# decisionforce/pgdrive

Measured on AMD Instinct MI355X. Metric: env-steps/sec (whole node) at 4096 envs x 240 lidar beams, higher is better.
Workload: dtype f32; 1 GPU; C3: 4096 envs/GPU x (1 ego + 16 IDM traffic slots) x 240 lidar beams, PGDrive-v0 maps seeds 1000-1099, uniform(-1,1) actions, auto-reset; step_kernel=k_step: one env per wave, specialised for the default single-agent configuration, envs_per_gpu=4096, global_envs=4096, obs_dim=274, engines_per_gpu=1, env_groups=1, parallelism=env-sharded dp1, no data-path collective, backend=none, steady_state=pre-roll 10000 steps (floor 10000), 1571 timed steps in 3 windows

## Files before the change

### pgdrive_amd/csrc/pgd_localize.h

```cpp
#ifndef PGD_LOCALIZE_H
#define PGD_LOCALIZE_H

DEV int cell_first(int c) { return c & 0xffffff; }
DEV int cell_mid(int c) { return (c & 0xffffff) + (int)((unsigned)c >> 24); }

template <class MV>
DEV float ray_grid(const MV& mv, float px, float py, float dx, float dy, unsigned kinds) {
  const float inv = 1.0f / mv.cell();
  int ix = (int)floorf((px - mv.ox()) * inv), iy = (int)floorf((py - mv.oy()) * inv);
  const int sx = dx > 0.0f ? 1 : -1, sy = dy > 0.0f ? 1 : -1;
  const float big = 3.0e38f;
  const float tdx = dx != 0.0f ? fabsf(mv.cell() / dx) : big, tdy = dy != 0.0f ? fabsf(mv.cell() / dy) : big;
  float tmx = dx != 0.0f ? ((mv.ox() + (ix + (dx > 0.0f ? 1 : 0)) * mv.cell()) - px) / dx : big;
  float tmy = dy != 0.0f ? ((mv.oy() + (iy + (dy > 0.0f ? 1 : 0)) * mv.cell()) - py) / dy : big;
  float best = 1.0f, t_enter = 0.0f;
  for (int it = 0; it < 64; ++it) {
    if (t_enter > best + 0.02f) break;
    if (ix >= 0 && iy >= 0 && ix < mv.gx() && iy < mv.gy()) {
      const int cell = iy * mv.gx() + ix;
      const int k1 = cell_first(mv.cstart[cell + 1]);
      for (int k = cell_mid(mv.cstart[cell]); k < k1; ++k) {
        const pgd_box b = mv.cbox[k];
        if (!((1u << b.kind) & kinds)) continue;
        best = fminf(best, ray_obb(obb_of(b), px, py, dx, dy));
      }
    } else if ((sx > 0 ? ix >= mv.gx() : ix < 0) || (sy > 0 ? iy >= mv.gy() : iy < 0)) {
      break;
    }
    if (tmx < tmy) { t_enter = tmx; tmx += tdx; ix += sx; }
    else { t_enter = tmy; tmy += tdy; iy += sy; }
    if (t_enter > 1.0f) break;
  }
  return best;
}


template <class MV>
DEV int cell_entry(const MV& mv, float px, float py) {
  int cx = (int)floorf((px - mv.ox()) / mv.cell()), cy = (int)floorf((py - mv.oy()) / mv.cell());
  return (cx >= 0 && cy >= 0 && cx < mv.gx() && cy < mv.gy()) ? mv.cstart[cy * mv.gx() + cx] : 0;
}

DEV int get_current_lane(const MapView& mv, const Grp& g, int c, float px, float py, float hx, float hy, int road_cur,
                         int road_next) {
  const int k0 = cell_first(c), k1 = cell_mid(c);
  unsigned best_cur = 0xffffffffu, best_next = 0xffffffffu, best_any = 0xffffffffu;
  const int stride = g.SUB;
  constexpr int NB = 3;
  for (int k = k0 + g.sub; k < k1; k += NB * stride) {
    pgd_box b[NB];
    LaneExt x[NB];
#pragma unroll
    for (int j = 0; j < NB; ++j) {
      int kk = k + j * stride;
      kk = kk < k1 ? kk : k;
      b[j] = mv.cbox[kk];
      x[j] = mv.cext[kk];
    }
#pragma unroll
    for (int j = 0; j < NB; ++j) {
      int kk = k + j * stride;
      if (kk >= k1) continue;
      if (!point_in_obb(obb_of(b[j]), px, py)) continue;
      unsigned key = ((unsigned)(kk - k0) << 16) | (unsigned)b[j].lane;
      bool is_cur = x[j].road == road_cur, is_next = x[j].road == road_next;
      if (!(key < best_any || (is_cur && key < best_cur) || (is_next && key < best_next))) continue;
      float dirx, diry;
      if (x[j].dir == 0.0f) { dirx = x[j].ax; diry = x[j].ay; }
      else { dirx = -x[j].dir * (py - x[j].ay); diry = x[j].dir * (px - x[j].ax); }
      if (!(dirx * hx + diry * hy > 0.0f)) continue;
      best_any = min(best_any, key);
      if (is_cur) best_cur = min(best_cur, key);
      if (is_next) best_next = min(best_next, key);
    }
  }
  best_cur = group_min(best_cur, g);
  best_next = group_min(best_next, g);
  best_any = group_min(best_any, g);
  unsigned pick = best_cur != 0xffffffffu ? best_cur : (road_next < 0 ? best_any : (best_next != 0xffffffffu ? best_next : best_any));
  return pick == 0xffffffffu ? -1 : (int)(pick & 0xffffu);
}

DEV void route_refresh(const MapView& mv, const pgd_spawn& sp, Veh& r) {
  const int rc = sp.ckpt_road[r.ck0], rn = sp.ckpt_road[r.ck1];
  r.road_cur = (uint32_t)rc; r.road_next = (uint32_t)rn;
  r.blk = 0; r.cur_first = 0; r.cur_n = 0; r.next_first = 0; r.next_n = 0;
  if (rc >= 0) {
    const pgd_road& CR = mv.roads()[rc];
    r.blk = CR.block_id; r.cur_first = CR.first_lane; r.cur_n = CR.n_lanes;
  }
  if (rn >= 0) {
    const pgd_road& NR = mv.roads()[rn];
    r.next_first = NR.first_lane; r.next_n = NR.n_lanes;
  }
}

#define PGD_CKPT_END (-32768)
DEV void update_checkpoints(const MapView& mv, const Grp& g, const pgd_spawn& sp, Veh& r, float lon, const int start_node) {
  if (r.ck0 == r.ck1) return;
  if (!(lon < 5.0f)) return;
  unsigned hit = 0xffffffffu;
  const int step = g.SUB;
#ifdef PGD_CKPT_CHAIN
  const int n = sp.n_ckpt;
  const int start_node_ = mv.roads()[mv.lanes[r.lane].road].from;
  for (int k = r.ck1 + g.sub; k < n - 1; k += 4 * step) {
    int v[4];
#pragma unroll
    for (int j = 0; j < 4; ++j) v[j] = sp.ckpt[min(k + j * step, n - 2)];
#pragma unroll
    for (int j = 0; j < 4; ++j)
      if (k + j * step < n - 1 && v[j] == start_node_) hit = min(hit, (unsigned)(k + j * step));
  }
#else
  for (int k = r.ck1 + g.sub; k < PGD_MAX_CKPT; k += 4 * step) {
    int v[4];
#pragma unroll
    for (int j = 0; j < 4; ++j) v[j] = sp.ckpt[min(k + j * step, PGD_MAX_CKPT - 1)];
#pragma unroll
    for (int j = 0; j < 4; ++j)
      if (k + j * step < PGD_MAX_CKPT && v[j] == start_node) hit = min(hit, (unsigned)(k + j * step));
    if (v[3] == PGD_CKPT_END) break;
  }
#endif
  hit = group_min(hit, g);
  if (hit == 0xffffffffu) return;
  const int idx = (int)hit;
  const int n_nodes = sp.n_ckpt;
  r.ck0 = idx;
  r.ck1 = (idx + 1 == n_nodes - 1) ? idx : idx + 1;
  route_refresh(mv, sp, r);
}

template <class MV>
DEV void update_localization(const MV& mv, const Grp& g, const pgd_spawn& sp, Veh& r, float& lon_out, float& lat_out,
                             const pgd_lane& PL) {
  const float s = r.hy, c = r.hx;
  const int road_cur = (int)r.road_cur;
  const int road_next = (r.ck0 == r.ck1) ? -1 : (int)r.road_next;
  PHASE_MARK(16);
  float lon = 0.0f, lat = 0.0f;
  bool stay = false;
  const int cell = cell_entry(mv, r.x, r.y);
  {
    if (PL.road == road_cur) {
      lane_local(PL, r.x, r.y, lon, lat);
      const float hw = 0.5f * PL.width;
      if (PL.dir == 0.0f) {
        stay = lon >= 0.0f && lon <= PL.length && lat <= hw + 0.55f && lat >= (PL.index > 0 ? 0.65f - hw : -hw - 0.55f) &&
               PL.bx * c + PL.by * s > 0.0f;
      } else {
        const int n = (int)(PL.length * 0.25f);
        const float r_in = PL.bx - PL.width - 1.0f;
        if (n >= 1 && r_in > 4.0f) {
          const float seg = PL.length / (float)n;
          const float dev = seg * seg / (4.0f * r_in) * 1.1f + 0.05f;
          float lo = -hw - 0.6f + dev;
          if (PL.index > 0) {
            const float nl = mv.lanes[r.lane - 1].length;
            const int nn = (int)(nl * 0.25f);
            if (nn >= 1) {
              const float nseg = nl / (float)nn;
              lo = fmaxf(lo, 0.6f - hw + nseg * nseg / (4.0f * r_in) * 1.1f + 0.05f);
            }
          }
          const float tx = -PL.dir * (r.y - PL.ay), ty = PL.dir * (r.x - PL.ax);
          stay = lon >= 0.0f && lon <= PL.length && lat <= hw + 0.6f - dev && lat >= lo && tx * c + ty * s > 0.0f;
        }
      }
    }
  }
  int lane = r.lane;
  if (!stay) lane = get_current_lane(mv, g, cell, r.x, r.y, c, s, road_cur, road_next);
  PHASE_MARK(17);
  bool on_lane = lane >= 0;
  if (!on_lane) lane = r.lane;
  r.lane = lane;
  int from_node = PL.pad;
  if (!stay) {
    const pgd_lane& NL = mv.lanes[lane];
    from_node = NL.pad;
    lane_local(NL, r.x, r.y, lon, lat);
  }
  lon_out = lon; lat_out = lat;
  r.lon = lon;
  update_checkpoints(mv, g, sp, r, lon, from_node);
  r.vflags = on_lane ? (r.vflags & ~PGD_F_OFF_LANE) : (r.vflags | PGD_F_OFF_LANE);
  PHASE_MARK(18);
}

template <class MV>
DEV unsigned state_check_part(const MV& mv, const int g_sub, const int g_SUB, const Obb& car) {
  float ex = fabsf(car.ux) * car.hl + fabsf(car.uy) * car.hw, ey = fabsf(car.uy) * car.hl + fabsf(car.ux) * car.hw;
  int cx0 = max((int)floorf((car.cx - ex - mv.ox()) / mv.cell()), 0), cx1 = min((int)floorf((car.cx + ex - mv.ox()) / mv.cell()), mv.gx() - 1);
  int cy0 = max((int)floorf((car.cy - ey - mv.oy()) / mv.cell()), 0), cy1 = min((int)floorf((car.cy + ey - mv.oy()) / mv.cell()), mv.gy() - 1);
  unsigned fl = 0;
  for (int cyb = cy0; cyb <= cy1; cyb += 2)
    for (int cxb = cx0; cxb <= cx1; cxb += 2) {
      int k0[4], pre[5];
      pre[0] = 0;
#pragma unroll
      for (int q = 0; q < 4; ++q) {
        int cx = cxb + (q & 1), cy = cyb + (q >> 1);
        bool in = cx <= cx1 && cy <= cy1;
        int cell = in ? cy * mv.gx() + cx : 0;
        int a = cell_mid(mv.cstart[cell]), b = cell_first(mv.cstart[cell + 1]);
        k0[q] = a;
        pre[q + 1] = pre[q] + (in ? b - a : 0);
      }
      const int n = pre[4];
      for (int f = g_sub; f < n; f += 2 * g_SUB) {
        pgd_box b[2];
        bool have[2];
#pragma unroll
        for (int j = 0; j < 2; ++j) {
          const int fj = f + j * g_SUB;
          have[j] = fj < n;
          const int ff = have[j] ? fj : f;
          const int q = (ff >= pre[1]) + (ff >= pre[2]) + (ff >= pre[3]);
          const int kk = (q == 0 ? k0[0] : q == 1 ? k0[1] : q == 2 ? k0[2] : k0[3]) + ff - (q == 0 ? pre[0] : q == 1 ? pre[1] : q == 2 ? pre[2] : pre[3]);
          b[j] = mv.cbox[kk];
        }
#pragma unroll
        for (int j = 0; j < 2; ++j) {
          if (!have[j]) continue;
          const unsigned bit = b[j].kind == PGD_BOX_WHITE ? PGD_F_ON_WHITE
                               : b[j].kind == PGD_BOX_YELLOW ? PGD_F_ON_YELLOW
                               : b[j].kind == PGD_BOX_BROKEN ? PGD_F_ON_BROKEN : PGD_F_CRASH_SIDEWALK;
          if (fl & bit) continue;
          if (obb_overlap(car, obb_of(b[j]))) fl |= bit;
        }
      }
    }
  return fl;
}
template <class MV>
DEV unsigned state_check(const MV& mv, const Grp& g, const Obb& car) { return group_or(state_check_part(mv, g.sub, g.SUB, car), g); }

struct RouteCtx {
  float drive;
  float positive;
  int clear;
  int lane_road;
};

template <bool AHEAD = false, class MV>
DEV void after_step_vehicle(const pgd_config& cfg, const MV& mv, const Grp& g, const pgd_spawn& sp, const pgd_spawn& sv, Veh& r,
                            bool is_agent, bool with_state_check, RouteCtx& ctx) {
  float lon_v, lat_v;
  const int lane0 = r.lane, first0 = (int)r.cur_first;
  const pgd_lane PL = mv.lanes[lane0];
  pgd_lane L0;
  if (AHEAD && is_agent) L0 = mv.lanes[first0];
  update_localization(mv, g, sp, r, lon_v, lat_v, PL);
  if (is_agent) {
    ctx = RouteCtx{0.0f, 1.0f, 0, -1};
    pgd_lane VL = PL;
    if (!AHEAD || r.lane != lane0) VL = mv.lanes[r.lane];
    ctx.lane_road = VL.road;
    if (!AHEAD || (int)r.cur_first != first0) L0 = mv.lanes[r.cur_first];
    {
      if (VL.dir == 0.0f && VL.ex > 0.0f) {
        const float ca = fabsf(r.hx * VL.bx + r.hy * VL.by), sa = fabsf(r.hy * VL.bx - r.hx * VL.by);
        const float hl = 0.5f * sv.length, hw = 0.5f * sv.width;
        const float e_lat = hw * ca + hl * sa, e_lon = hl * ca + hw * sa;
        ctx.clear = (fabsf(lat_v) + e_lat <= VL.ex && lon_v - e_lon >= 0.0f && lon_v + e_lon <= VL.length) ? 1 : 0;
      }
    }
    unsigned fl = (unsigned)r.vflags;
    fl &= ~(PGD_F_ON_WHITE | PGD_F_ON_YELLOW | PGD_F_ON_BROKEN | PGD_F_CRASH_SIDEWALK | PGD_F_OUT_OF_ROUTE);
    if (with_state_check && !ctx.clear) fl |= state_check(mv, g, Obb{r.x, r.y, r.hx, r.hy, 0.5f * sv.length, 0.5f * sv.width});
    float lon, lat;
    lane_local(L0, r.x, r.y, lon, lat);
    float w = mv.lane_width();
    r.dl = lat + w * 0.5f;
    float range = w * (float)r.cur_n;
    if (r.blk == 'y' || r.blk == 'Y') {
      float sx, sy;
      lane_position(L0, lon, -0.5f * L0.width, sx, sy);
      range = 50.0f * ray_grid(mv, sx, sy, -L0.by * 50.0f, L0.bx * 50.0f, (1u << PGD_BOX_WHITE) | (1u << PGD_BOX_YELLOW));
    }
    r.dr = range - r.dl;
    {
      const bool in_ref = VL.road == (int)r.road_cur;
      float l0, t0;
      lane_local(in_ref ? VL : L0, r.lastx, r.lasty, l0, t0);
      const float l1 = in_ref ? lon_v : lon, t1 = in_ref ? lat_v : lat;
      ctx.positive = (in_ref || (cfg.marl_flags & PGD_MA_PLAIN_REWARD)) ? 1.0f : (mv.roads()[VL.road].negative ? -1.0f : 1.0f);
      const float lateral_factor = cfg.use_lateral ? clipf(1.0f - 2.0f * fabsf(t1) / w, 0.0f, 1.0f) : 1.0f;
      ctx.drive = cfg.driving_reward * (l1 - l0) * lateral_factor * ctx.positive;
    }
    if (r.dr < 0.0f || r.dl < 0.0f) fl |= PGD_F_OUT_OF_ROUTE;
    r.vflags = (int)fl;
    float dist = norm2(r.lastx - r.x, r.lasty - r.y) / 1000.0f;
    r.energy += 3.25f * expf(0.01f * speed_kmh(r.v)) * dist / 100.0f * 1000.0f;
    PHASE_MARK(19);
  }
}

template <class MV>
DEV unsigned state_check_wave(const MV& mv, const Obb& car) {
  const int lane = threadIdx.x;
  float ex = fabsf(car.ux) * car.hl + fabsf(car.uy) * car.hw, ey = fabsf(car.uy) * car.hl + fabsf(car.ux) * car.hw;
  int cx0 = max((int)floorf((car.cx - ex - mv.ox()) / mv.cell()), 0), cx1 = min((int)floorf((car.cx + ex - mv.ox()) / mv.cell()), mv.gx() - 1);
  int cy0 = max((int)floorf((car.cy - ey - mv.oy()) / mv.cell()), 0), cy1 = min((int)floorf((car.cy + ey - mv.oy()) / mv.cell()), mv.gy() - 1);
  unsigned fl = 0;
  for (int cyb = cy0; cyb <= cy1; cyb += 2)
    for (int cxb = cx0; cxb <= cx1; cxb += 2) {
      int k0[4], pre[5];
      pre[0] = 0;
#pragma unroll
      for (int q = 0; q < 4; ++q) {
        int cx = cxb + (q & 1), cy = cyb + (q >> 1);
        bool in = cx <= cx1 && cy <= cy1;
        int cell = in ? cy * mv.gx() + cx : 0;
        int a = cell_mid(mv.cstart[cell]), b = cell_first(mv.cstart[cell + 1]);
        k0[q] = a;
        pre[q + 1] = pre[q] + (in ? b - a : 0);
      }
      for (int f = lane; f < pre[4]; f += WAVE) {
        int q = (f >= pre[1]) + (f >= pre[2]) + (f >= pre[3]);
        int kk = (q == 0 ? k0[0] : q == 1 ? k0[1] : q == 2 ? k0[2] : k0[3]) + f - (q == 0 ? pre[0] : q == 1 ? pre[1] : q == 2 ? pre[2] : pre[3]);
        pgd_box b = mv.cbox[kk];
        unsigned bit = b.kind == PGD_BOX_WHITE ? PGD_F_ON_WHITE
                       : b.kind == PGD_BOX_YELLOW ? PGD_F_ON_YELLOW
                       : b.kind == PGD_BOX_BROKEN ? PGD_F_ON_BROKEN : PGD_F_CRASH_SIDEWALK;
        if (obb_overlap(car, obb_of(b))) fl |= bit;
      }
    }
  unsigned out = 0;
  if (__ballot((fl & PGD_F_ON_WHITE) != 0)) out |= PGD_F_ON_WHITE;
  if (__ballot((fl & PGD_F_ON_YELLOW) != 0)) out |= PGD_F_ON_YELLOW;
  if (__ballot((fl & PGD_F_ON_BROKEN) != 0)) out |= PGD_F_ON_BROKEN;
  if (__ballot((fl & PGD_F_CRASH_SIDEWALK) != 0)) out |= PGD_F_CRASH_SIDEWALK;
  return out;
}

#endif
```

### pgdrive_amd/csrc/pgd_step.h

```cpp
#define WAVE 64
#define MAXV 64

#ifndef PGD_MA_PRIO3
#define PGD_MA_PRIO3 7
#define PGD_MA_PRIO2 5
#define PGD_MA_PRIO1 3
#endif
#ifdef PGD_PROF
#define PROF_BLOCKS 8192
__device__ unsigned long long g_phase_cycles[PROF_BLOCKS * 32];
__shared__ long long s_prof_t0, s_prof_w0;
#define PHASE_MARK(k)                                                                                      \
  do {                                                                                                     \
    if ((int)threadIdx.x == __builtin_ffsll((long long)__ballot(1)) - 1 && blockIdx.x < PROF_BLOCKS) {       \
      long long _now = clock64();                                                                          \
      g_phase_cycles[blockIdx.x * 32 + (k)] += (unsigned long long)(_now - s_prof_t0);                     \
      s_prof_t0 = _now;                                                                                    \
    }                                                                                                      \
  } while (0)
#define PHASE_INIT() do { if (threadIdx.x == 0) { s_prof_t0 = clock64(); s_prof_w0 = wall_clock64(); } } while (0)
#define PHASE_END_AT(k) do { if (threadIdx.x == 0 && blockIdx.x < PROF_BLOCKS) g_phase_cycles[blockIdx.x * 32 + (k)] += (unsigned long long)(wall_clock64() - s_prof_w0); } while (0)
#define PHASE_END() PHASE_END_AT(15)
#elif defined(PGD_EXITAT)
#define PHASE_MARK(k)
// ... 171 lines not shown
  float lk_klat, lk_khead, lk_vt, lk_noise;
  uint32_t lk_tick;
};
template <bool ONE_ENV, bool MARL, bool OBJ, bool STD = false, int FIX = 0, bool LK = false>
__global__ __launch_bounds__(WAVE, PGD_WAVES_PER_SIMD) void k_step(PgdDev d, const float* __restrict__ act, float* __restrict__ reward,
                                                uint8_t* __restrict__ done, uint32_t* __restrict__ flags,
                                                float* __restrict__ obs, const PgdCold cold) {
  if (FIX) write_fixed_config<ONE_ENV, MARL, STD, FIX>(d);

  __shared__ StepUnion U;
  Snap& S = U.step.S;
  ObsScratch& OU = U.step.OU;
  ObsLds& OL = OU.ol;
  SubPose& SUBP = OU.sp;
  __shared__ AgentView s_ag[FUSE_MAX_AGENTS];
  __shared__ int s_flag[WAVE];
  __shared__ int s_hit[WAVE];
  __shared__ int s_aux;
  __shared__ uint8_t s_kind[WAVE];
  const int V = d.V, A = d.A, N = d.N;
  const int lane = threadIdx.x;
  const bool sub_ok = (ONE_ENV ? V : d.epw * V) <= PGD_SUBV;
  const int unit = (int)blockIdx.x + d.unit_off;
  const LaneMap lm = lane_map(d, unit, N);
  const int el = ONE_ENV ? 0 : lm.el, s = lm.s, e = ONE_ENV ? unit : lm.e, base = ONE_ENV ? 0 : lm.base;
  const bool valid = lm.valid, leader = lm.sub == 0;
  const Grp g{lm.sub, d.sub, lm.lead};
  const int slot = base + s;

  PHASE_INIT();
  XMARK(99);
  Veh r;
  RouteCtx ctx{0.0f, 1.0f, 0, -1};
  using MV = typename std::conditional<FIX != 0 && !OBJ, MapViewPre, MapView>::type;
  MV mv;
  const pgd_spawn* sp = nullptr;
  constexpr bool FIXE_K = FIX != 0 && !ONE_ENV && !MARL && !STD;
  constexpr bool REGSP = ONE_ENV || FIXE_K;
  pgd_spawn sl;
  pgd_lane FL;
#define SPV spawn_ref<REGSP>(sl, sp)
  const pgd_scenario* sc = nullptr;
  int ng = 0, ep_steps = 0;
  uint32_t steps_total = 0;
  bool near_env = true;
  int trig_hint = 0;
#ifdef PGD_NO_SUBSTEP
  constexpr bool n_mid_enabled = false;
#else
  constexpr bool n_mid_enabled = true;
#endif
  S.present[lane] = 0;
  s_flag[lane] = 0;
  s_hit[lane] = 0;
  if (lane < PGD_SUBV) SUBP.trav[lane] = 0.0f;
  constexpr bool one_env = ONE_ENV;
  constexpr bool marl = MARL;
  int scen = 0;
  unsigned long long im = 0ull;
  const bool packed = !ONE_ENV && d.pack_obs != 0;
  const bool own_first = FIX == 0 && ONE_ENV && !d.use_imask;
  if (own_first && valid) load_rec(rec_block(d.rec, (size_t)e, V), V, s, r);
  if ((ONE_ENV || (packed && valid)) && d.use_imask) im = d.imask[e];
  if (one_env || valid) scen = d.ei[(size_t)e * PGD_NEI + EI_SCEN];
  constexpr bool LATE_WORDS = MARL && FIX != 0;
  int hint_early = 0;
  if (LATE_WORDS && (one_env || valid)) hint_early = d.ei[(size_t)e * PGD_NEI + EI_NEAR];
  if (valid && !own_first) load_rec(((ONE_ENV || packed) && ((im >> s) & 1ull)) ? rec_block(d.reset_img, (size_t)scen, V) : rec_block(d.rec, (size_t)e, V), V, s, r);
  float2 act_in = make_float2(0.0f, 0.0f);
  constexpr bool ACT_EARLY = ONE_ENV || FIXE_K;
  if (ACT_EARLY && valid && s < A) {
    if (LK) {
      const float* o = cold.lk_obs + ((size_t)e * A + s) * d.D;
      const float2 q0 = *reinterpret_cast<const float2*>(o), q1 = *reinterpret_cast<const float2*>(o + 2);
      act_in = lane_keep_action(cold.seed, cold.env_base + e, q0.x, q0.y, q1.x, q1.y, cold.lk_klat, cold.lk_khead, cold.lk_vt, cold.lk_noise, cold.lk_tick);
    } else act_in = *reinterpret_cast<const float2*>(act + ((size_t)e * A + s) * 2);
  }
  constexpr bool EARLY_HEAD = !MARL && REGSP && FIX != 0 && !OBJ;
  if (EARLY_HEAD && valid) { sp = d.spawns + (size_t)scen * d.sstride + s; spawn_head_load<false>(sp, sl); }
  const int key0 = valid ? (r.status ^ (r.vflags << 3)) : 0;
  auto env_words = [&]() {
    ng = d.ei[(size_t)(e) * PGD_NEI + EI_NEXT_GROUP];
    ep_steps = d.ei[(size_t)(e) * PGD_NEI + EI_EP_STEPS];
    steps_total = (uint32_t)d.ei[(size_t)(e) * PGD_NEI + EI_STEPS_TOTAL];
    if (ONE_ENV || packed) {
      const int hint = d.ei[(size_t)(e) * PGD_NEI + EI_NEAR];
      near_env = (hint & 1) != 0;
      trig_hint = (hint >> 1) & 3;
    }
  };
  if (one_env || valid) {
    sc = d.scen + scen;
    mv = map_view_as<MV>(d, d.env_map + e);
    if (!LATE_WORDS) env_words();
  }
  PHASE_MARK(13);
  XMARK(13);
  if (valid) {
    if (!EARLY_HEAD || (int)r.spawn != s) {
      sp = d.spawns + (size_t)scen * d.sstride + r.spawn;
      if (REGSP) spawn_head_load<MARL>(sp, sl);
    }
    if (marl && r.status == ST_DYING && --r.timer == 0) r.status = ST_EMPTY;
  }
  if (LATE_WORDS && (ONE_ENV || packed)) { near_env = (hint_early & 1) != 0; trig_hint = (hint_early >> 1) & 3; }
  bool on_trigger;
  if (ONE_ENV && !MARL && A == 1 && trig_hint != 0) on_trigger = valid && s < A && trig_hint == 2;
  else if ((MARL || FIXE_K) && d.no_groups) on_trigger = false;
  else on_trigger = valid && s < A && r.status == ST_ACTIVE && ng < sc->n_groups && mv.lanes[r.lane].road == sc->trigger_road[ng];
  bool trig;
  if (ONE_ENV) {
    trig = __ballot(on_trigger) != 0ull;
  } else {
    step_sync();
    if (on_trigger) s_flag[el] = 1;
    step_sync();
    trig = valid && s_flag[el] != 0;
  }
  PHASE_MARK(0);
  XMARK(0);
  if (valid && trig && r.status == ST_PENDING && SPV.group == ng) r.status = ST_ACTIVE;
  if (trig) ng += 1;
  int next_trigger_road = -1;
  if (ONE_ENV && !MARL && A == 1) next_trigger_road = ng < sc->n_groups ? (int)sc->trigger_road[ng] : -1;
  const bool idm_ego = !MARL && d.cfg.idm_agent != 0;
  const bool idm_runs = ONE_ENV ? (__ballot(valid && (s >= A || idm_ego) && r.status == ST_ACTIVE) != 0ull) : true;
  if (valid) {
    if (leader) {
      S.x[slot] = r.x; S.y[slot] = r.y; S.ux[slot] = r.hx; S.uy[slot] = r.hy;
      S.spd[slot] = speed_kmh(r.v);
      const int kind = OBJ ? (int)SPV.kind : PGD_OBJ_VEHICLE;
      if (OBJ) s_kind[slot] = kind;
      S.hl[slot] = 0.5f * SPV.length; S.hw[slot] = kind == PGD_OBJ_CYLINDER ? -1.0f : 0.5f * SPV.width;
      S.lane[slot] = r.lane;
      const bool present = r.status == ST_PENDING || r.status == ST_ACTIVE || r.status == ST_DYING;
      S.present[slot] = present ? 1 : 0;
      if (present && (V > A || idm_ego) && idm_runs) {
        const pgd_lane& ml = mv.lanes[r.lane];
        S.lon[slot] = r.lon;
        S.llen[slot] = ml.length;
        S.succ[slot] = *reinterpret_cast<const int4*>(ml.succ);
      }
    }
  }
  step_sync();
  PHASE_MARK(1);
  XMARK(1);
  const bool acting = valid && r.status == ST_ACTIVE;
  if (ONE_ENV) {
    const int nact = __popcll(__ballot(acting && leader && s >= A));
    if (MARL && V == A) {
      const int nag = __popcll(__ballot(acting && leader));
      if (nag * 10 >= A * PGD_MA_PRIO3) __builtin_amdgcn_s_setprio(3);
      else if (nag * 10 >= A * PGD_MA_PRIO2) __builtin_amdgcn_s_setprio(2);
      else if (nag * 10 >= A * PGD_MA_PRIO1) __builtin_amdgcn_s_setprio(1);
    } else
    if (nact >= 4) __builtin_amdgcn_s_setprio(3);
    else if (nact >= 2) __builtin_amdgcn_s_setprio(2);
    else if (nact > 0) __builtin_amdgcn_s_setprio(1);
  }
  if (acting) {
    float st, tb;
    if (s < A && !idm_ego) {
      float a0 = ACT_EARLY ? act_in.x : act[((size_t)e * A + s) * 2 + 0], a1 = ACT_EARLY ? act_in.y : act[((size_t)e * A + s) * 2 + 1];
      if (a0 != a0) a0 = 0.0f;
      if (a1 != a1) a1 = 0.0f;
      st = clipf(a0, -1.0f, 1.0f);
      tb = clipf(a1, -1.0f, 1.0f);
      if (d.cfg.discrete_action) {
        st = st * (2.0f / (float)(d.cfg.discrete_steering_dim - 1)) - 1.0f;
        tb = tb * (2.0f / (float)(d.cfg.discrete_throttle_dim - 1)) - 1.0f;
      }
    } else {
#ifdef PGD_NO_IDM
      st = 0.0f; tb = 0.0f;
#else
      idm_act<OBJ>(d, mv, g, SPV, S, base, V, s, e, steps_total, r, st, tb);
#endif
    }
    PHASE_MARK(2);
    r.vflags &= ~(PGD_F_CRASH_VEHICLE | PGD_F_CRASH_OBJECT | PGD_F_CRASH_BUILDING);
    r.lastx = r.x; r.lasty = r.y;
    r.lasthx = r.hx; r.lasthy = r.hy;
    r.a0s = r.a1s; r.a0t = r.a1t;
    r.a1s = st; r.a1t = tb;
    r.steer = (s < A && d.cfg.increment_steering) ? clipf(r.steer + st * 0.05f, -1.0f, 1.0f)
              : ((d.cfg.idm_steer_lag > 0.0f && (s >= A || idm_ego))
                     ? r.steer + (clipf(st, -1.0f, 1.0f) - r.steer) * ((d.cfg.dt * (float)d.cfg.decision_repeat) / (d.cfg.idm_steer_lag + d.cfg.dt * (float)d.cfg.decision_repeat))
                     : st);
    dynamics(d, SPV, r, s < A && d.cfg.enable_reverse != 0, tb, leader ? &SUBP : nullptr, slot, near_env && sub_ok && n_mid_enabled);
    PHASE_MARK(3);
  }
  step_sync();
  if (acting && leader) { S.x[slot] = r.x; S.y[slot] = r.y; S.ux[slot] = r.hx; S.uy[slot] = r.hy; }
  step_sync();
#ifdef PGD_NO_SUBSTEP
  const int n_mid = 0;
#else
  const int n_mid = (d.cfg.decision_repeat <= PGD_MAX_SUB && sub_ok) ? d.cfg.decision_repeat - 1 : 0;
#endif
  if (near_env) {
    const int my_kind = (OBJ && valid) ? s_kind[slot] : PGD_OBJ_VEHICLE;
    constexpr bool PAIR_LISTS = ONE_ENV && MARL && !OBJ;
    auto pair_touch = [&](const int bs, const int as, const Obb& me, const float my_trav, const Obb& ag, const float ag_trav) {
      bool hit = shape_overlap<OBJ, PAIR_LISTS>(ag, me);
      for (int k = 0; k < n_mid && !hit; ++k) {
        Obb ak = ag, mk = me;
        if (ag_trav > 0.0f) {
          const float4 q = SUBP.p[k][as]; const float2 b = SUBP.beta[as];
          ak.cx = q.x; ak.cy = q.y; ak.ux = q.z * b.x + q.w * b.y; ak.uy = q.w * b.x - q.z * b.y;
        }
        if (my_trav > 0.0f) {
          const float4 q = SUBP.p[k][bs]; const float2 b = SUBP.beta[bs];
          mk.cx = q.x; mk.cy = q.y; mk.ux = q.z * b.x + q.w * b.y; mk.uy = q.w * b.x - q.z * b.y;
        }
        hit = shape_overlap<OBJ, PAIR_LISTS>(ak, mk);
      }
      return hit;
    };
    const bool by_mask = ONE_ENV && MARL && !OBJ && A > g.SUB;
    if (by_mask) {
      constexpr int CAP = 736;
      static_assert(2 * CAP + WAVE <= (int)(sizeof(float) * 2 * WAVE + sizeof(int4) * WAVE), "pair list + body list live in Snap::lon .. succ");
      unsigned short* plist = reinterpret_cast<unsigned short*>(&S.lon[0]);
      unsigned char* bl = reinterpret_cast<unsigned char*>(plist + CAP);
      const bool body = valid && leader && S.present[slot] != 0;
      const unsigned long long bm = __ballot(body);
      const int n = __popcll(bm);
      const bool any_agent = __ballot(body && s < A && acting) != 0ull;
      if (n >= 2 && any_agent) {
        if (body) bl[__popcll(bm & ((1ull << lane) - 1ull))] = (unsigned char)(slot | ((s < A && acting) ? 0x80 : 0));
        step_sync();
        const int K = n <= WAVE / 2 ? WAVE / n : 1, half = n / 2;
        const int k = lane / n, i = lane - k * n;
        const bool lane_on = k < K;
        const int ei = bl[lane_on ? i : 0], bi = ei & 0x3f;
        const Obb me = snap_obb(S, bi);
        const float my_trav = sub_ok ? SUBP.trav[bi] : 0.0f;
        const float my_reach = me.hl + (me.hw < 0.0f ? 0.0f : me.hw) + my_trav + 0.01f;
        int count = 0;
        auto flush = [&]() {
          step_sync();
          for (int p0 = 0; p0 < count; p0 += WAVE) {
            const int p = p0 + lane;
            if (p < count) {
              const int pr = plist[p], bs = pr >> 8, as = pr & 0xff;
              if (pair_touch(bs, as, snap_obb(S, bs), sub_ok ? SUBP.trav[bs] : 0.0f, snap_obb(S, as), sub_ok ? SUBP.trav[as] : 0.0f)) {
                s_hit[bs] = 1; s_hit[as] = 1;
              }
            }
          }
          step_sync();
          count = 0;
        };
        for (int r0 = 1; r0 <= half; r0 += K) {
          const int r = r0 + k;
          int j = i + r;
          j -= j >= n ? n : 0;
          const bool pair_on = lane_on && r <= half && !(2 * r == n && i >= half);
          const int ej = bl[pair_on ? j : 0], bj = ej & 0x3f;
          const float ox = S.x[bj], oy = S.y[bj], ohl = S.hl[bj], ohw = S.hw[bj];
          const float o_trav = sub_ok ? SUBP.trav[bj] : 0.0f;
          const float reach = my_reach + ohl + (ohw < 0.0f ? 0.0f : ohw) + o_trav;
          const float ddx = ox - me.cx, ddy = oy - me.cy;
          const bool within = pair_on && ((ei | ej) & 0x80) != 0 && !(ddx * ddx + ddy * ddy > reach * reach);
          const unsigned long long wm = __ballot(within);
          if (within) plist[count + __popcll(wm & ((1ull << lane) - 1ull))] = (unsigned short)((bi << 8) | bj);
          count += __popcll(wm);
          if (count > CAP - WAVE) flush();
        }
        if (count > 0) flush();
      }
    } else
    if (valid && S.present[slot]) {
      const Obb me = snap_obb(S, slot);
      const float my_trav = sub_ok ? SUBP.trav[slot] : 0.0f;
      const float my_rad = me.hl + (me.hw < 0.0f ? 0.0f : me.hw);
      const bool live = !OBJ || my_kind == PGD_OBJ_VEHICLE || !(r.vflags & (int)PGD_F_OBJECT_HIT);
      bool touched = false;
      const bool split = !OBJ || my_kind == PGD_OBJ_VEHICLE;
      for (int a = split ? g.sub : 0; a < A; a += split ? g.SUB : 1) {
        if (a == s || (OBJ && !S.present[base + a])) continue;
        const Obb ag = snap_obb(S, base + a);
        const float ag_trav = sub_ok ? SUBP.trav[base + a] : 0.0f;
        const float reach = my_rad + ag.hl + ag.hw + my_trav + ag_trav + 0.01f;
        const float ddx = ag.cx - me.cx, ddy = ag.cy - me.cy;
        if (ddx * ddx + ddy * ddy > reach * reach) continue;
        if (!pair_touch(slot, base + a, me, my_trav, ag, ag_trav)) continue;
        touched = true;
        if (!OBJ) s_hit[base + a] = 1;
        else if ((leader || split) && live) atomicOr(&s_hit[base + a], my_kind == PGD_OBJ_VEHICLE ? 1 : (my_kind == PGD_OBJ_BUILDING ? 4 : 2));
      }
      if (OBJ && touched && my_kind != PGD_OBJ_VEHICLE && my_kind != PGD_OBJ_BUILDING) r.vflags |= (int)PGD_F_OBJECT_HIT;
    }
    step_sync();
    if (acting && s < A) {
      if (s_hit[slot] & 1) r.vflags |= PGD_F_CRASH_VEHICLE;
      if (OBJ && (s_hit[slot] & 2)) r.vflags |= PGD_F_CRASH_OBJECT;
      if (OBJ && (s_hit[slot] & 4)) r.vflags |= PGD_F_CRASH_BUILDING;
    }
  }
  PHASE_MARK(4);
  XMARK(4);
  if (acting) {
    if (REGSP && FIX && !OBJ && s < A) FL = mv.lanes[SPV.dest_lane];
    after_step_vehicle<ONE_ENV>(d.cfg, mv, g, *sp, SPV, r, s < A, !one_env, ctx);
    if (s >= A && (r.vflags & PGD_F_OFF_LANE)) r.status = ST_REMOVED;
  }
  int trig_next = 0;
  if (ONE_ENV && !MARL && A == 1 && valid && s < A)
    trig_next = (r.status == ST_ACTIVE && next_trigger_road >= 0 && ctx.lane_road == next_trigger_road) ? 2 : 1;
  if (one_env && A > 1) {
    const bool need = acting && s < A && !ctx.clear;
    const unsigned long long need_m = __ballot(need && leader);
    if (d.sub > 3) {
      if (need) r.vflags |= (int)state_check(mv, g, Obb{r.x, r.y, r.hx, r.hy, 0.5f * SPV.length, 0.5f * SPV.width});
    } else if (need_m != 0ull) {
      unsigned char* nl = reinterpret_cast<unsigned char*>(&S.lon[0]);
      unsigned* fo = reinterpret_cast<unsigned*>(&S.llen[0]);
      const int n_need = __popcll(need_m);
      const int my_pos = __popcll(need_m & ((1ull << (need ? g.lead : 0)) - 1ull));
      if (need && leader) nl[my_pos] = (unsigned char)slot;
      fo[lane] = 0u;
      step_sync();
      const int G = WAVE / n_need, gi = lane / G;
      if (gi < n_need) {
        const unsigned part = state_check_part(mv, lane - gi * G, G, snap_obb(S, nl[gi]));
        if (part != 0u) atomicOr(&fo[gi], part);
      }
      step_sync();
      if (need) r.vflags |= (int)fo[my_pos];
    }
  }
  PHASE_MARK(25);
  if (one_env && A == 1) {
    if (__ballot(leader && valid && s < A && acting && !ctx.clear) != 0ull) {
      unsigned fl = state_check_wave(mv, snap_obb(S, 0));
      if (valid && s == 0) r.vflags |= (int)fl;
    }
  }
  PHASE_MARK(5);
  XMARK(5);
  if (LATE_WORDS && (one_env || valid)) {
    asm volatile("" ::: "memory");
    ng = d.ei[(size_t)(e) * PGD_NEI + EI_NEXT_GROUP];
    ep_steps = d.ei[(size_t)(e) * PGD_NEI + EI_EP_STEPS];
    steps_total = (uint32_t)d.ei[(size_t)(e) * PGD_NEI + EI_STEPS_TOTAL];
  }
  ep_steps += 1;
  steps_total += 1;
  bool want_reset = false;
  if (!ONE_ENV) {
    s_flag[lane] = 0;
    step_sync();
  }
  unsigned my_fl = 0;
  bool fresh = false;
  int fresh_idx = 0, fresh_id = 0;
  bool my_dn = false;
  float my_rew = 0.0f;
  const bool was_active = acting;
  if (valid && s < A && !marl) {
    if (r.status == ST_ACTIVE) my_rew = reward_done<false>(d, mv, SPV, dest_lane_ref<REGSP && FIX != 0 && !OBJ>(FL, mv.lanes, SPV.dest_lane), r, ctx, my_fl, my_dn);
    if (d.cfg.horizon > 0 && ep_steps >= d.cfg.horizon) { my_dn = true; my_fl |= PGD_F_MAX_STEP; }
    if (sc->max_steps > 0 && ep_steps >= sc->max_steps) { my_dn = true; my_fl |= PGD_F_MAX_STEP; }
    r.eprew += my_rew;
    bool will_reset = my_dn && d.cfg.auto_reset && A == 1;
    if (will_reset) { my_fl |= PGD_F_RESET; want_reset = true; if (!ONE_ENV) s_flag[el] = 1; }
  }
  if (marl && one_env) {
    const pgd_config& gcf = d.cfg;
    const bool toll = (gcf.marl_flags & PGD_MA_TOLLGATE) != 0;
    const bool parking = (gcf.marl_flags & PGD_MA_PARKING) != 0;
    if (parking && lane == 0) s_aux = d.ei[(size_t)e * PGD_NEI + EI_AUX];
    if (parking) step_sync();
    if (valid && s < A && was_active) {
      if (toll && r.blk == '$') r.php += 1.0f;
      my_rew = reward_done<true>(d, mv, SPV, dest_lane_ref<REGSP && FIX != 0>(FL, mv.lanes, SPV.dest_lane), r, ctx, my_fl, my_dn);
      const bool arrive = my_fl & PGD_F_ARRIVE, oor = my_fl & PGD_F_OUT_OF_ROAD, crash = my_fl & PGD_F_CRASH_VEHICLE;
      if (crash && !(gcf.marl_flags & PGD_MA_CRASH_DONE) && !(arrive || oor)) my_dn = false;
      if (oor && !(gcf.marl_flags & PGD_MA_OUT_ROAD_DONE) && !arrive) my_dn = false;
      if (toll && r.phi >= 0.0f && r.plp >= 0.0f && r.plp - r.phi < (float)gcf.min_pass_steps) {
        my_dn = true;
        my_fl |= PGD_F_OUT_OF_ROAD;
      }
      if (r.rlane < 0x7fff) r.rlane += 1;
      if (gcf.horizon > 0 && r.rlane >= gcf.horizon) { my_dn = true; my_fl |= PGD_F_MAX_STEP; }
      r.eprew += my_rew;
      my_fl |= PGD_F_REPORT;
      if (my_dn && parking && r.php > 0.0f) {
        if (leader) atomicOr(&s_aux, 1 << ((int)r.php - 1));
        r.php = 0.0f;
      }
      if (my_dn) {
        if (arrive || gcf.delay_done <= 0) r.status = ST_EMPTY;
        else { r.status = ST_DYING; r.timer = gcf.delay_done; }
      }
    }
    if (valid && leader && s < A) {
      const size_t k = (size_t)e * A + s;
      reward[k] = my_rew;
      done[k] = my_dn ? 1 : 0;
      if (d.prow) {
        float* tail = d.prow + (size_t)e * d.ostride + (size_t)A * d.D;
        tail[s] = my_rew;
        tail[A + s] = my_dn ? 1.0f : 0.0f;
      }
    }
    PHASE_MARK(26);
    step_sync();
    if (valid && leader) {
      S.x[slot] = r.x; S.y[slot] = r.y; S.ux[slot] = r.hx; S.uy[slot] = r.hy;
      S.hl[slot] = 0.5f * SPV.length; S.hw[slot] = 0.5f * SPV.width;
      S.present[slot] = (r.status == ST_PENDING || r.status == ST_ACTIVE || r.status == ST_DYING) ? 1 : 0;
    }
    step_sync();
    const bool is_lead_agent = valid && leader && s < A;
    int alive = __popcll(__ballot(is_lead_agent && (r.status == ST_ACTIVE || r.status == ST_DYING)));
    int next_agent = d.ei[(size_t)e * PGD_NEI + EI_NEXT_AGENT];
    const bool allow = (gcf.marl_flags & PGD_MA_ALLOW_RESPAWN) && !(gcf.horizon > 0 && ep_steps >= gcf.horizon) &&
                       alive < gcf.agent_limit;
    if (allow) {
      const pgd_spawn* rbase = d.spawns + (size_t)scen * d.sstride + V;
      unsigned long long freem = 0ull;
      float plx = 0.0f, ply = 0.0f, plc = 1.0f, pls = 0.0f;
      if (lane < gcf.respawn_places) {
        const pgd_spawn& place = rbase[lane * gcf.respawn_dests];
        const float2 phv = cold.spawn_hv[(size_t)scen * d.sstride + V + lane * gcf.respawn_dests];
        plx = place.x; ply = place.y; plc = phv.x; pls = phv.y;
      }
      const Obb mine = snap_obb(S, lane < V ? lane : 0);
      const bool here = lane < V && S.present[lane];
      for (int p = 0; p < gcf.respawn_places; ++p) {
        const Obb region{__shfl(plx, p), __shfl(ply, p), __shfl(plc, p), __shfl(pls, p), 4.0f, 1.5f};
        const bool blocks = here && obb_overlap(region, mine);
        if (__ballot(blocks) == 0ull) freem |= 1ull << p;
      }
      const unsigned long long em = __ballot(is_lead_agent && r.status == ST_EMPTY && !(my_fl & PGD_F_REPORT));
      const unsigned pool = parking ? ((unsigned)s_aux & ((1u << gcf.respawn_dests) - 1u)) : 1u;
      if (freem != 0ull && em != 0ull && __ballot(pool != 0u) != 0ull) {
        int kth = (int)(pgd_rng(gcf.seed, (uint32_t)(gcf.env_base + e), 0x51ace5u, (uint32_t)next_agent) % (uint32_t)__popcll(freem));
        unsigned long long fm = freem;
        while (kth-- > 0) fm &= fm - 1ull;
        const int p = __builtin_ffsll((long long)fm) - 1;
        const int src = __builtin_ffsll((long long)em) - 1;
        const int tslot = (src / d.sub) % V;
        int dest = (int)(pgd_rng(gcf.seed, (uint32_t)(gcf.env_base + e), 0x0a9e47u + (uint32_t)p, (uint32_t)next_agent) %
                         (uint32_t)gcf.respawn_dests);
        if (parking) {
          int pick = (int)(pgd_rng(gcf.seed, (uint32_t)(gcf.env_base + e), 0x0a9e47u + (uint32_t)p, (uint32_t)next_agent) %
                           (uint32_t)__popc(pool));
          dest = 0;
          for (int b = 0; b < 32; ++b)
            if (pool & (1u << b)) { if (pick-- == 0) { dest = b; break; } }
          step_sync();
          if (lane == 0) s_aux &= ~(1 << dest);
        }
        if (valid && s == tslot) {
          fresh_idx = V + p * gcf.respawn_dests + dest;
          fresh_id = next_agent;
          fresh = true;
          my_fl |= PGD_F_NEW;
          if (leader) {
            const pgd_spawn& nsp = d.spawns[(size_t)scen * d.sstride + fresh_idx];
            const float2 nhv = cold.spawn_hv[(size_t)scen * d.sstride + fresh_idx];
            S.x[slot] = nsp.x; S.y[slot] = nsp.y; S.ux[slot] = nhv.x; S.uy[slot] = nhv.y;
            S.hl[slot] = 0.5f * nsp.length; S.hw[slot] = 0.5f * nsp.width;
            S.present[slot] = 1;
          }
        }
        next_agent += 1;
        step_sync();
      }
    }
    if (fresh) {
      sp = d.spawns + (size_t)scen * d.sstride + fresh_idx;
      if (REGSP) spawn_head_load<MARL>(sp, sl);
      load_rec(rec_block(cold.respawn_img, (size_t)scen, d.sstride - V), d.sstride - V, fresh_idx - V, r);
      r.agent_id = (float)fresh_id;
    }
    PHASE_MARK(27);
    if (toll && valid && s < A && r.status == ST_ACTIVE) {
      const float cur = (float)r.blk, last = r.pli;
      r.pli = cur;
      if (last >= 0.0f && last != cur) {
        if (r.blk == '$') r.phi = (float)ep_steps;
        else if ((r.blk == 'y' || r.blk == 'Y') && last == (float)'$') r.plp = (float)ep_steps;
      }
    }
    const int n_active = __popcll(__ballot(is_lead_agent && r.status == ST_ACTIVE));
    const bool all_done = n_active == 0 || (gcf.horizon > 0 && ep_steps >= 5 * gcf.horizon);
    if (all_done) {
      my_fl |= PGD_F_ALL_DONE;
      if (gcf.auto_reset) { my_fl |= PGD_F_RESET; want_reset = true; }
    }
    if (lane == 0) d.ei[(size_t)e * PGD_NEI + EI_NEXT_AGENT] = next_agent;
    if (parking) {
      step_sync();
      if (lane == 0) d.ei[(size_t)e * PGD_NEI + EI_AUX] = s_aux;
    }
  }
  if (!ONE_ENV) step_sync();
  PHASE_MARK(6);
  XMARK(6);
  int episodes = 0;
  const bool resetting = ONE_ENV ? (__ballot(want_reset) != 0ull) : (valid && s_flag[el]);
  if (resetting) {
    episodes = d.ei[(size_t)(e) * PGD_NEI + EI_EPISODES] + 1;
    if (d.cfg.resample_scenario)
      scen = (int)(pgd_rng(cold.seed, (uint32_t)(cold.env_base + e), 0x5ce9a210u, (uint32_t)episodes) % (uint32_t)cold.n_scen);
    sc = d.scen + scen;
    mv = map_view_as<MV>(d, cold.scen_map + scen);
    ng = 0;
    ep_steps = 0;
  }
  if (valid && resetting) {
    sp = d.spawns + (size_t)scen * d.sstride + s;
    if (REGSP) spawn_head_load<MARL>(sp, sl);
    load_rec(rec_block(d.reset_img, (size_t)scen, V), V, s, r);
    const unsigned long long am = __ballot(leader && s < A && r.status == ST_ACTIVE);
    if (marl && s < A && r.status == ST_ACTIVE) my_fl |= PGD_F_NEW;
    if (s == 0 && d.cfg.resample_scenario)
      for (int q = g.sub; q < (int)(sizeof(pgd_map) / 16); q += g.SUB)
        reinterpret_cast<uint4*>(d.env_map + e)[q] = reinterpret_cast<const uint4*>(cold.scen_map + scen)[q];
    if (s == 0 && leader) {
      d.ei[(size_t)(e) * PGD_NEI + EI_SCEN] = scen;
      d.ei[(size_t)(e) * PGD_NEI + EI_EPISODES] = episodes;
      d.ei[(size_t)(e) * PGD_NEI + EI_NEXT_AGENT] = A == 1 ? 1 : __popcll(am);
      d.ei[(size_t)(e) * PGD_NEI + EI_AUX] = sc->aux;
      if (cold.bev_fill) cold.bev_fill[e] = 1;
    }
  }
  if (valid && leader && s < A) {
    size_t k = (size_t)e * A + s;
    flags[k] = my_fl;
    if (!marl) {
      reward[k] = my_rew;
      done[k] = my_dn ? 1 : 0;
      if (d.prow) {
        float* tail = d.prow + (size_t)e * d.ostride + (size_t)A * d.D;
        tail[s] = my_rew;
        tail[A + s] = my_dn ? 1.0f : 0.0f;
      }
    }
  }
  PHASE_MARK(7);
  XMARK(7);
  bool stored = false;
  if (valid && leader) {
    stored = acting || resetting || (r.status ^ (r.vflags << 3)) != key0 || (key0 & 7) == ST_DYING;
    if (stored) store_veh(d, e, s, r);
    if (s == 0) {
      d.ei[(size_t)(e) * PGD_NEI + EI_NEXT_GROUP] = ng;
      d.ei[(size_t)(e) * PGD_NEI + EI_EP_STEPS] = ep_steps;
      d.ei[(size_t)(e) * PGD_NEI + EI_STEPS_TOTAL] = (int)steps_total;
    }
  }
  if (ONE_ENV) {
    const unsigned long long sb = __ballot(stored);
    const unsigned long long cleared = __ballot(lane < V && ((sb >> (lane * d.sub)) & 1ull) != 0ull);
    const unsigned long long full = V >= 64 ? ~0ull : ((1ull << V) - 1ull);
    const unsigned long long nm = resetting ? full : (im & ~cleared);
    if (lane == 0 && nm != im && d.use_imask) d.imask[e] = nm;
  } else if (packed) {
    const unsigned long long sb = __ballot(stored);
    const unsigned long long full = (1ull << V) - 1ull;
    const unsigned long long nm = resetting ? full : (im & ~((sb >> base) & full));
    if (valid && s == 0 && nm != im && d.use_imask) d.imask[e] = nm;
  }
  PHASE_MARK(8);
  XMARK(8);
  bool near_next = true;
  if (ONE_ENV && !MARL && obs != nullptr) {
    step_sync();
    if (valid && leader) {
      const bool present = r.status == ST_PENDING || r.status == ST_ACTIVE || r.status == ST_DYING;
      S.x[slot] = r.x; S.y[slot] = r.y; S.ux[slot] = r.hx; S.uy[slot] = r.hy;
      S.spd[slot] = r.status == ST_DYING ? 0.0f : speed_kmh(r.v);
      S.hl[slot] = 0.5f * SPV.length;
      S.hw[slot] = (OBJ && SPV.kind == PGD_OBJ_CYLINDER) ? -1.0f : 0.5f * SPV.width;
      if (OBJ) s_kind[slot] = SPV.kind;
      S.present[slot] = present ? 1 : 0;
      if (s < A) {
        AgentView& ag = s_ag[s];
        ag.x = r.x; ag.y = r.y; ag.th = r.th; ag.hx = r.hx; ag.hy = r.hy; ag.dl = r.dl; ag.dr = r.dr; ag.v = r.v;
        ag.steer = r.steer; ag.a0s = r.a0s; ag.a0t = r.a0t; ag.lhx = r.lasthx; ag.lhy = r.lasthy;
        ag.cur_first = r.cur_first; ag.cur_n = r.cur_n; ag.next_first = r.next_first;
        ag.blk = r.blk; ag.toll_time = r.php;
        ag.env = e; ag.slot = s; ag.tick = steps_total;
      }
    }
    step_sync();
    const int scen_now = scen;
    const MV& mvo = mv;
    PHASE_MARK(20);
  XMARK(20);
    bool near_any = false;
    const float t_step = d.cfg.dt * (float)d.cfg.decision_repeat;
    for (int a = 0; a < A; ++a) {
      const AgentView ag = s_ag[a];
      const bool have = lane < V && d.cfg.num_lasers > 0;
      bool near_a = false;
      ObsPre pre;
      obs_preload(d, mvo, ag, lane, WAVE, pre);
      obs_compact<OBJ>(OL, lane, a, have && S.present[lane], OBJ ? (have && s_kind[lane] == PGD_OBJ_VEHICLE) : true, S.x[lane], S.y[lane],
                  S.ux[lane], S.uy[lane], S.hl[lane], S.hw[lane], S.spd[lane], ag.x, ag.y, d.cfg.lidar_dist, ag.hx, ag.hy,
                  d.cfg.num_lasers, S.hl[a] + S.hw[a] + near_reach(ag.v, t_step), &near_a, t_step);
      near_any = near_any || near_a;
      step_sync();
      PHASE_MARK(21);
// ... 110 lines not shown
```

### pgdrive_amd/csrc/pgd_vehicle.h

```cpp
#ifndef PGD_VEHICLE_H
#define PGD_VEHICLE_H

DEV const RecPiece* rec_block(const RecPiece* base, size_t block, int n) { return base + block * (size_t)(8 * n); }
DEV RecPiece* rec_block(RecPiece* base, size_t block, int n) { return base + block * (size_t)(8 * n); }
DEV void load_rec(const RecPiece* blk, int n, int s, Veh& r) {
  uint4* dst = reinterpret_cast<uint4*>(&r);
#pragma unroll
  for (int k = 0; k < 8; ++k) dst[k] = blk[k * n + s].q;
}
DEV void load_rec_head(const RecPiece* blk, int n, int s, Veh& r) {
  uint4* dst = reinterpret_cast<uint4*>(&r);
#pragma unroll
  for (int k = 0; k < 4; ++k) dst[k] = blk[k * n + s].q;
}
DEV void store_rec(RecPiece* blk, int n, int s, const Veh& r) {
  const uint4* src = reinterpret_cast<const uint4*>(&r);
#pragma unroll
  for (int k = 0; k < 8; ++k) blk[k * n + s].q = src[k];
}
DEV uint32_t rec_word(const RecPiece* blk, int n, int s, int w) { return reinterpret_cast<const uint32_t*>(blk + (w >> 2) * n + s)[w & 3]; }
DEV float rec_float(const RecPiece* blk, int n, int s, int w) { return __uint_as_float(rec_word(blk, n, s, w)); }
enum { RW_X = 0, RW_Y = 1, RW_TH = 2, RW_LANE_SPAWN = 8 };
DEV int rec_spawn(const RecPiece* blk, int n, int s) { return (int)(rec_word(blk, n, s, RW_LANE_SPAWN) >> 16); }
DEV void load_veh(const PgdDev& d, int e, int s, Veh& r) { load_rec(rec_block(d.rec, (size_t)e, d.V), d.V, s, r); }
DEV void store_veh(const PgdDev& d, int e, int s, const Veh& r) { store_rec(rec_block(d.rec, (size_t)e, d.V), d.V, s, r); }

DEV float speed_kmh(float v) { return clipf(fabsf(v) * 3.6f, 0.0f, 100000.0f); }

struct Snap {
  float x[WAVE], y[WAVE], ux[WAVE], uy[WAVE], spd[WAVE], hl[WAVE], hw[WAVE];
  int lane[WAVE], present[WAVE];
  float lon[WAVE], llen[WAVE];
  int4 succ[WAVE];
};
DEV bool succ_has(const int4& p, int id) {
  unsigned u = (unsigned)id & 0xffffu;
  unsigned a = (unsigned)p.x, b = (unsigned)p.y, c = (unsigned)p.z, d = (unsigned)p.w;
  return (a & 0xffffu) == u || (a >> 16) == u || (b & 0xffffu) == u || (b >> 16) == u || (c & 0xffffu) == u ||
         (c >> 16) == u || (d & 0xffffu) == u || (d >> 16) == u;
}
DEV Obb snap_obb(const Snap& S, int k) { return Obb{S.x[k], S.y[k], S.ux[k], S.uy[k], S.hl[k], S.hw[k]}; }

#define PGD_MAX_SUB 5
#ifndef PGD_SUBV
#define PGD_SUBV 52
#endif
struct SubPose {
  float4 p[PGD_MAX_SUB - 1][PGD_SUBV];
  float2 beta[PGD_SUBV];
  float trav[PGD_SUBV];
};

struct Grp {
  int sub, SUB, lead;
};
DEV unsigned group_min(unsigned v, const Grp& g) {
  if (g.SUB <= 4) {
    const int m = g.SUB - 1;
    const unsigned a = (unsigned)__shfl((int)v, g.lead), b = (unsigned)__shfl((int)v, g.lead + min(1, m)),
                   c = (unsigned)__shfl((int)v, g.lead + min(2, m)), e = (unsigned)__shfl((int)v, g.lead + m);
    return min(min(a, b), min(c, e));
  }
  unsigned r = v;
  for (int j = 0; j < g.SUB; ++j) r = min(r, (unsigned)__shfl((int)v, g.lead + j));
  return r;
}
DEV unsigned group_or(unsigned v, const Grp& g) {
  if (g.SUB <= 4) {
    const int m = g.SUB - 1;
    const unsigned a = (unsigned)__shfl((int)v, g.lead), b = (unsigned)__shfl((int)v, g.lead + min(1, m)),
                   c = (unsigned)__shfl((int)v, g.lead + min(2, m)), e = (unsigned)__shfl((int)v, g.lead + m);
    return a | b | c | e;
  }
  unsigned r = v;
  for (int j = 0; j < g.SUB; ++j) r |= (unsigned)__shfl((int)v, g.lead + j);
  return r;
}

#endif
```

Measured before the change: 240.8 million env-steps/s.

## Redistribute lane-box scan across the whole wave for vehicles needing relocalization

Splits vehicle post-step localization into a head (stay check), an optional lane search, and a tail. In the single-env configuration, vehicles that leave their lane are compacted into a list in shared Snap scratch, and the whole wave's lanes are divided among them to scan cell boxes. Per-walker minima are then combined with shared-memory atomicMin instead of group shuffles. This targets load imbalance when only a few vehicles need a full lane search, at the cost of extra wave syncs, scratch reuse of Snap fields, and atomics.

```diff
diff --git a/pgdrive_amd/csrc/pgd_localize.h b/pgdrive_amd/csrc/pgd_localize.h
--- a/pgdrive_amd/csrc/pgd_localize.h
+++ b/pgdrive_amd/csrc/pgd_localize.h
@@ -41,13 +41,11 @@
   return (cx >= 0 && cy >= 0 && cx < mv.gx() && cy < mv.gy()) ? mv.cstart[cy * mv.gx() + cx] : 0;
 }
 
-DEV int get_current_lane(const MapView& mv, const Grp& g, int c, float px, float py, float hx, float hy, int road_cur,
-                         int road_next) {
+DEV void lane_box_scan(const MapView& mv, int c, int sub, int stride, float px, float py, float hx, float hy, int road_cur, int road_next,
+                       unsigned& best_cur, unsigned& best_next, unsigned& best_any) {
   const int k0 = cell_first(c), k1 = cell_mid(c);
-  unsigned best_cur = 0xffffffffu, best_next = 0xffffffffu, best_any = 0xffffffffu;
-  const int stride = g.SUB;
   constexpr int NB = 3;
-  for (int k = k0 + g.sub; k < k1; k += NB * stride) {
+  for (int k = k0 + sub; k < k1; k += NB * stride) {
     pgd_box b[NB];
     LaneExt x[NB];
 #pragma unroll
@@ -74,11 +72,55 @@
       if (is_next) best_next = min(best_next, key);
     }
   }
+}
+DEV int lane_pick(unsigned best_cur, unsigned best_next, unsigned best_any, int road_next) {
+  unsigned pick = best_cur != 0xffffffffu ? best_cur : (road_next < 0 ? best_any : (best_next != 0xffffffffu ? best_next : best_any));
+  return pick == 0xffffffffu ? -1 : (int)(pick & 0xffffu);
+}
+
+DEV int get_current_lane(const MapView& mv, const Grp& g, int c, float px, float py, float hx, float hy, int road_cur,
+                         int road_next) {
+  unsigned best_cur = 0xffffffffu, best_next = 0xffffffffu, best_any = 0xffffffffu;
+  lane_box_scan(mv, c, g.sub, g.SUB, px, py, hx, hy, road_cur, road_next, best_cur, best_next, best_any);
   best_cur = group_min(best_cur, g);
   best_next = group_min(best_next, g);
   best_any = group_min(best_any, g);
-  unsigned pick = best_cur != 0xffffffffu ? best_cur : (road_next < 0 ? best_any : (best_next != 0xffffffffu ? best_next : best_any));
-  return pick == 0xffffffffu ? -1 : (int)(pick & 0xffffu);
+  return lane_pick(best_cur, best_next, best_any, road_next);
+}
+
+DEV int lane_walk_wave(const MapView& mv, Snap& S, const Grp& g, int slot, bool need, unsigned long long need_m, int cell, int road_cur,
+                       int road_next) {
+  int* w_slot = reinterpret_cast<int*>(&S.lon[0]);
+  int* w_cell = reinterpret_cast<int*>(&S.llen[0]);
+  unsigned* w_road = reinterpret_cast<unsigned*>(&S.succ[0]);
+  unsigned* w_min = w_road + WAVE;
+  static_assert(sizeof(int4) * WAVE >= sizeof(unsigned) * 4 * WAVE, "roads + three minima per walker live in Snap::succ");
+  const int lane = threadIdx.x;
+  const int n = __popcll(need_m);
+  const int my_pos = __popcll(need_m & ((1ull << (need ? g.lead : 0)) - 1ull));
+  if (need && g.sub == 0) {
+    w_slot[my_pos] = slot; w_cell[my_pos] = cell;
+    w_road[my_pos] = ((unsigned)road_cur & 0xffffu) | ((unsigned)road_next << 16);
+    w_min[3 * my_pos] = 0xffffffffu; w_min[3 * my_pos + 1] = 0xffffffffu; w_min[3 * my_pos + 2] = 0xffffffffu;
+  }
+  wave_sync();
+  const int G = WAVE / n, gi = lane / G;
+  if (gi < n) {
+    const int ws = w_slot[gi], c = w_cell[gi];
+    const unsigned roads = w_road[gi];
+    const int rc = (int)(roads & 0xffffu), rn = (int)roads >> 16;
+    unsigned best_cur = 0xffffffffu, best_next = 0xffffffffu, best_any = 0xffffffffu;
+    lane_box_scan(mv, c, lane - gi * G, G, S.x[ws], S.y[ws], S.ux[ws], S.uy[ws], rc, rn, best_cur, best_next, best_any);
+    if (best_any != 0xffffffffu) {
+      atomicMin(&w_min[3 * gi + 2], best_any);
+      if (best_cur != 0xffffffffu) atomicMin(&w_min[3 * gi], best_cur);
+      if (best_next != 0xffffffffu) atomicMin(&w_min[3 * gi + 1], best_next);
+    }
+  }
+  wave_sync();
+  int pick = -1;
+  if (need) pick = lane_pick(w_min[3 * my_pos], w_min[3 * my_pos + 1], w_min[3 * my_pos + 2], road_next);
+  return pick;
 }
 
 DEV void route_refresh(const MapView& mv, const pgd_spawn& sp, Veh& r) {
@@ -132,16 +174,22 @@
   route_refresh(mv, sp, r);
 }
 
-template <class MV>
-DEV void update_localization(const MV& mv, const Grp& g, const pgd_spawn& sp, Veh& r, float& lon_out, float& lat_out,
-                             const pgd_lane& PL) {
+struct LocStage {
+  float lon, lat;
+  int cell;
+  int road_cur, road_next;
+  bool stay = true;
+};
+template <class MV>
+DEV void localize_stay(const MV& mv, const Veh& r, const pgd_lane& PL, LocStage& st) {
   const float s = r.hy, c = r.hx;
   const int road_cur = (int)r.road_cur;
-  const int road_next = (r.ck0 == r.ck1) ? -1 : (int)r.road_next;
+  st.road_cur = road_cur;
+  st.road_next = (r.ck0 == r.ck1) ? -1 : (int)r.road_next;
   PHASE_MARK(16);
   float lon = 0.0f, lat = 0.0f;
   bool stay = false;
-  const int cell = cell_entry(mv, r.x, r.y);
+  st.cell = cell_entry(mv, r.x, r.y);
   {
     if (PL.road == road_cur) {
       lane_local(PL, r.x, r.y, lon, lat);
@@ -170,14 +218,18 @@
       }
     }
   }
-  int lane = r.lane;
-  if (!stay) lane = get_current_lane(mv, g, cell, r.x, r.y, c, s, road_cur, road_next);
-  PHASE_MARK(17);
+  st.lon = lon; st.lat = lat; st.stay = stay;
+}
+template <class MV>
+DEV void localize_finish(const MV& mv, const Grp& g, const pgd_spawn& sp, Veh& r, float& lon_out, float& lat_out, const pgd_lane& PL,
+                         const LocStage& st, int lane) {
+  float lon = st.lon, lat = st.lat;
+  if (st.stay) lane = r.lane;
   bool on_lane = lane >= 0;
   if (!on_lane) lane = r.lane;
   r.lane = lane;
   int from_node = PL.pad;
-  if (!stay) {
+  if (!st.stay) {
     const pgd_lane& NL = mv.lanes[lane];
     from_node = NL.pad;
     lane_local(NL, r.x, r.y, lon, lat);
@@ -244,15 +296,26 @@
   int lane_road;
 };
 
+struct AfterStage {
+  pgd_lane PL, L0;
+  int lane0, first0;
+  LocStage loc;
+};
 template <bool AHEAD = false, class MV>
-DEV void after_step_vehicle(const pgd_config& cfg, const MV& mv, const Grp& g, const pgd_spawn& sp, const pgd_spawn& sv, Veh& r,
-                            bool is_agent, bool with_state_check, RouteCtx& ctx) {
+DEV void after_step_head(const MV& mv, const Veh& r, bool is_agent, AfterStage& as) {
+  as.lane0 = r.lane; as.first0 = (int)r.cur_first;
+  as.PL = mv.lanes[as.lane0];
+  if (AHEAD && is_agent) as.L0 = mv.lanes[as.first0];
+  localize_stay(mv, r, as.PL, as.loc);
+}
+template <bool AHEAD = false, class MV>
+DEV void after_step_tail(const pgd_config& cfg, const MV& mv, const Grp& g, const pgd_spawn& sp, const pgd_spawn& sv, Veh& r,
+                         bool is_agent, bool with_state_check, RouteCtx& ctx, AfterStage& as, int lane) {
   float lon_v, lat_v;
-  const int lane0 = r.lane, first0 = (int)r.cur_first;
-  const pgd_lane PL = mv.lanes[lane0];
-  pgd_lane L0;
-  if (AHEAD && is_agent) L0 = mv.lanes[first0];
-  update_localization(mv, g, sp, r, lon_v, lat_v, PL);
+  const pgd_lane& PL = as.PL;
+  pgd_lane& L0 = as.L0;
+  const int lane0 = as.lane0, first0 = as.first0;
+  localize_finish(mv, g, sp, r, lon_v, lat_v, PL, as.loc, lane);
   if (is_agent) {
     ctx = RouteCtx{0.0f, 1.0f, 0, -1};
     pgd_lane VL = PL;
@@ -297,6 +360,16 @@
     PHASE_MARK(19);
   }
 }
+template <bool AHEAD = false, class MV>
+DEV void after_step_vehicle(const pgd_config& cfg, const MV& mv, const Grp& g, const pgd_spawn& sp, const pgd_spawn& sv, Veh& r,
+                            bool is_agent, bool with_state_check, RouteCtx& ctx) {
+  AfterStage as;
+  after_step_head<AHEAD>(mv, r, is_agent, as);
+  int lane = r.lane;
+  if (!as.loc.stay) lane = get_current_lane(mv, g, as.loc.cell, r.x, r.y, r.hx, r.hy, as.loc.road_cur, as.loc.road_next);
+  PHASE_MARK(17);
+  after_step_tail<AHEAD>(cfg, mv, g, sp, sv, r, is_agent, with_state_check, ctx, as, lane);
+}
 
 template <class MV>
 DEV unsigned state_check_wave(const MV& mv, const Obb& car) {
diff --git a/pgdrive_amd/csrc/pgd_step.h b/pgdrive_amd/csrc/pgd_step.h
--- a/pgdrive_amd/csrc/pgd_step.h
+++ b/pgdrive_amd/csrc/pgd_step.h
@@ -497,10 +497,30 @@
   }
   PHASE_MARK(4);
   XMARK(4);
+#ifdef PGD_LANE_WALK_GROUP
+  constexpr bool WAVE_WALK = false;
+#else
+  constexpr bool WAVE_WALK = ONE_ENV && !MARL;
+#endif
+  AfterStage as;
   if (acting) {
     if (REGSP && FIX && !OBJ && s < A) FL = mv.lanes[SPV.dest_lane];
-    after_step_vehicle<ONE_ENV>(d.cfg, mv, g, *sp, SPV, r, s < A, !one_env, ctx);
-    if (s >= A && (r.vflags & PGD_F_OFF_LANE)) r.status = ST_REMOVED;
+    if constexpr (WAVE_WALK) after_step_head<ONE_ENV>(mv, r, s < A, as);
+    else {
+      after_step_vehicle<ONE_ENV>(d.cfg, mv, g, *sp, SPV, r, s < A, !one_env, ctx);
+      if (s >= A && (r.vflags & PGD_F_OFF_LANE)) r.status = ST_REMOVED;
+    }
+  }
+  if constexpr (WAVE_WALK) {
+    const bool need_walk = acting && !as.loc.stay;
+    const unsigned long long walk_m = __ballot(need_walk && leader);
+    int lane_now = -1;
+    if (walk_m != 0ull) lane_now = lane_walk_wave(mv, S, g, slot, need_walk, walk_m, as.loc.cell, as.loc.road_cur, as.loc.road_next);
+    PHASE_MARK(17);
+    if (acting) {
+      after_step_tail<ONE_ENV>(d.cfg, mv, g, *sp, SPV, r, s < A, !one_env, ctx, as, lane_now);
+      if (s >= A && (r.vflags & PGD_F_OFF_LANE)) r.status = ST_REMOVED;
+    }
   }
   int trig_next = 0;
   if (ONE_ENV && !MARL && A == 1 && valid && s < A)
diff --git a/pgdrive_amd/csrc/pgd_vehicle.h b/pgdrive_amd/csrc/pgd_vehicle.h
--- a/pgdrive_amd/csrc/pgd_vehicle.h
+++ b/pgdrive_amd/csrc/pgd_vehicle.h
@@ -76,5 +76,9 @@
   for (int j = 0; j < g.SUB; ++j) r |= (unsigned)__shfl((int)v, g.lead + j);
   return r;
 }
+DEV void wave_sync() {
+  __builtin_amdgcn_fence(__ATOMIC_ACQ_REL, "wavefront");
+  __builtin_amdgcn_wave_barrier();
+}
 
 #endif
```

Result: no change. 241.6 million env-steps/s (median of 4 runs) (+0.3%).
